# dmMaze/comic-text-detector

Hardware: NVIDIA H100
Metric: pages/sec @1024x1024 synthetic (higher is better)
Workload: dtype fp16

## Files before the change

### comic-text-detector_b200/csrc/conv_tc.cu

```cuda
#include <cstdlib>
#include <cstring>
#include <cuda.h>
#include <cuda_fp16.h>
#include <cuda_runtime.h>

#include "kernels.h"
#include "ptx.cuh"

namespace ctd {

constexpr int kTileW = 16;
constexpr int kThreads = 384;

template <int BN, int TH>
struct TcCfg {
  static constexpr int kABytes = TH * kTileW * 128;
  static constexpr int kBBytes = BN * 128;
  static constexpr int kStages = TH == 8 ? (BN >= 128 ? 5 : (BN >= 64 ? 8 : 10))
                                         : (BN >= 128 ? 3 : (BN >= 64 ? 4 : (BN >= 32 ? 5 : 6)));
  static constexpr int kBoxN = BN < 64 ? BN : 64;
  static constexpr int kBoxBytes = 8 * TH * kBoxN * 2;
  static constexpr int kStgBytes = (BN / kBoxN) * kBoxBytes;
  static constexpr int kBiasFloats = 512;
  static constexpr size_t kSmem = 1024 + size_t(kStages) * (kABytes + kBBytes) + 2 * kStgBytes + 256 + kBiasFloats * 4;
  static_assert(kSmem <= 227 * 1024, "conv_tc_kernel: shared memory");
  static_assert(kBoxBytes % 1024 == 0, "conv_tc_kernel: store boxes must keep the 1024-byte swizzle alignment");
};

template <int ACT>
__device__ __forceinline__ float apply_act(float v) {
  if constexpr (ACT == CTD_ACT_SILU) return __fdividef(v, 1.0f + exp_neg_fast(v));
  else if constexpr (ACT == CTD_ACT_LEAKY) return fmaxf(v, 0.1f * v);
  else if constexpr (ACT == CTD_ACT_RELU) return fmaxf(v, 0.f);
  else if constexpr (ACT == CTD_ACT_SIGMOID) return __fdividef(1.0f, 1.0f + exp_neg_fast(v));
  else return v;
}

template <int ACT>
__device__ __forceinline__ float apply_act_precise(float v) {
  if constexpr (ACT == CTD_ACT_SILU) return v / (1.0f + expf(-v));
  else if constexpr (ACT == CTD_ACT_LEAKY) return fmaxf(v, 0.1f * v);
  else if constexpr (ACT == CTD_ACT_RELU) return fmaxf(v, 0.f);
  else if constexpr (ACT == CTD_ACT_SIGMOID) return 1.0f / (1.0f + expf(-v));
  else return v;
}

template <int BN>
__device__ __forceinline__ void wgmma_bn(float (&d)[BN / 2], uint64_t ad, uint64_t bd, uint32_t acc) {
  if constexpr (BN == 128) wgmma_n128(d, ad, bd, acc);
  else if constexpr (BN == 64) wgmma_n64(d, ad, bd, acc);
  else if constexpr (BN == 32) wgmma_n32(d, ad, bd, acc);
  else wgmma_n16(d, ad, bd, acc);
}

template <int BN, int TH, int ACT, bool RES>
__device__ __forceinline__ void stage_f16(const float (&acc)[BN / 2], const float* __restrict__ bias_s, uint32_t stg,
                                          int m, int warp4, int lane) {
  using Cfg = TcCfg<BN, TH>;
  constexpr uint32_t kRowBytes = Cfg::kBoxN * 2;
  const int q = lane >> 3;
  const uint32_t pixrow = uint32_t(m * 64 + warp4 * 16 + (q & 1) * 8 + (lane & 7));
#pragma unroll
  for (int j = 0; j < BN / 8; j += 2) {
    const int col = (j + (q >> 1)) * 8;
    const uint32_t off = pixrow * kRowBytes + uint32_t(col % Cfg::kBoxN) * 2;
    const uint32_t addr = stg + uint32_t(col / Cfg::kBoxN) * Cfg::kBoxBytes +
                          (off ^ (((off >> 7) & (kRowBytes / 16 - 1)) << 4));
    uint32_t r[4];
    if constexpr (RES) ldmatrix_x4(addr, r);
#pragma unroll
    for (int i = 0; i < 4; ++i) {
      const int c = (j + (i >> 1)) * 8 + (lane & 3) * 2;
      float f0 = apply_act<ACT>(acc[j * 4 + 2 * i] + bias_s[c]);
      float f1 = apply_act<ACT>(acc[j * 4 + 2 * i + 1] + bias_s[c + 1]);
      if constexpr (RES) {
        __half2 h;
        memcpy(&h, &r[i], 4);
        const float2 rv = __half22float2(h);
        f0 = __fadd_rn(f0, rv.x);
        f1 = __fadd_rn(f1, rv.y);
      }
      const __half2 o = __floats2half2_rn(f0, f1);
      memcpy(&r[i], &o, 4);
    }
    stmatrix_x4(addr, r);
  }
}

template <int ACT>
__device__ __forceinline__ void epi_pair_f32(float v0, float v1, const float* __restrict__ bias_s, int col,
                                             float* __restrict__ out, int ncols, bool residual) {
  if (col >= ncols) return;
  float f0 = apply_act_precise<ACT>(v0 + bias_s[col]);
  float f1 = apply_act_precise<ACT>(v1 + bias_s[col + 1]);
  if (col + 1 < ncols) {
    if (residual) {
      const float2 r = *reinterpret_cast<const float2*>(out + col);
      f0 += r.x;
      f1 += r.y;
    }
    *reinterpret_cast<float2*>(out + col) = make_float2(f0, f1);
  } else {
    if (residual) f0 += out[col];
    out[col] = f0;
  }
}

template <int BN, int ACT>
__device__ __forceinline__ void epilogue_f32(const float (&acc)[BN / 2], const float* __restrict__ bias_s,
                                             float* const (&out)[2], const bool (&valid)[2], int ncols, int lane,
                                             bool residual) {
#pragma unroll
  for (int h = 0; h < 2; ++h) {
    if (!valid[h]) continue;
#pragma unroll
    for (int j = 0; j < BN / 8; ++j)
      epi_pair_f32<ACT>(acc[j * 4 + 2 * h], acc[j * 4 + 2 * h + 1], bias_s, j * 8 + (lane & 3) * 2, out[h], ncols,
                        residual);
  }
// ... 167 lines not shown
      int prev = -1;
      for (int k_it = 0; k_it < its_per_tile; ++k_it) {
        mbar_wait(full_bar + 8 * stage, full_par);
        const uint64_t ad = a_desc0 + uint64_t(stage) * (Cfg::kABytes >> 4);
        const uint64_t bd = b_desc0 + uint64_t(stage) * (Cfg::kBBytes >> 4);
        wgmma_fence();
        for (int ks = 0; ks < ksteps; ++ks)
#pragma unroll
          for (int m = 0; m < MT; ++m)
            wgmma_bn<BN>(acc[m], ad + m * a_mstep + 2 * ks, bd + 2 * ks, (k_it > 0 || ks > 0) ? 1u : 0u);
        wgmma_commit();
        wgmma_wait<1>();
        if (prev >= 0 && wg_leader) mbar_arrive(empty_bar + 8 * prev);
        prev = stage;
        if (++stage == Cfg::kStages) { stage = 0; full_par ^= 1u; }
      }
      wgmma_wait<0>();
#pragma unroll
      for (int m = 0; m < MT; ++m) wgmma_fence_regs(acc[m]);
      if (prev >= 0 && wg_leader) mbar_arrive(empty_bar + 8 * prev);
    }

    const float* bias_t = bias_s + nblk * BN;
    if (nhwc16) {
      if (res16) {
        mbar_wait(res_bar, res_par);
        res_par ^= 1u;
      } else {
        if (wg_leader) tma_store_wait_read();
        named_barrier_sync(epi_bar, 128);
      }
#define CTD_EPI(ACT)                                                                                   \
  _Pragma("unroll") for (int m = 0; m < MT; ++m) {                                                     \
    if (res16) stage_f16<BN, TH, ACT, true>(acc[m], bias_t, stg, m, warp & 3, lane);                   \
    else stage_f16<BN, TH, ACT, false>(acc[m], bias_t, stg, m, warp & 3, lane);                        \
  }
      switch (g.act) {
        case CTD_ACT_SILU: CTD_EPI(CTD_ACT_SILU) break;
        case CTD_ACT_LEAKY: CTD_EPI(CTD_ACT_LEAKY) break;
        case CTD_ACT_RELU: CTD_EPI(CTD_ACT_RELU) break;
        case CTD_ACT_SIGMOID: CTD_EPI(CTD_ACT_SIGMOID) break;
        default: CTD_EPI(CTD_ACT_NONE) break;
      }
#undef CTD_EPI
      fence_proxy_async();
      named_barrier_sync(epi_bar, 128);
      if (wg_leader) {
#pragma unroll
        for (int b = 0; b < BN / Cfg::kBoxN; ++b)
          tma_store_4d(&p.d_map[phase], stg + b * Cfg::kBoxBytes, nblk * BN + b * Cfg::kBoxN, x0, sy0, img);
        tma_store_commit();
      }
      if (p.dst_map_cols < g.cout && p.dst_map_cols < (nblk + 1) * BN) {
#pragma unroll
        for (int m = 0; m < MT; ++m)
#pragma unroll
          for (int h = 0; h < 2; ++h) {
            const int row = (wg * MT + m) * 64 + wrow + 8 * h;
            const int gy = y0 + row / kTileW, gx = x0 + row % kTileW;
            if (gy >= g.gh || gx >= g.gw) continue;
            const int oy = gy * g.out_mul + (phase >> 1), ox = gx * g.out_mul + (phase & 1);
            __half* out = p.dst + (size_t(img) * g.dst_h * g.dst_w + size_t(oy) * g.dst_w + ox) * g.dst_cstride +
                          g.dst_coff;
#pragma unroll
            for (int i = 0; i < R; ++i) {
              if (((i >> 1) & 1) != h) continue;
              const int c = (i >> 2) * 8 + (lane & 3) * 2 + (i & 1), col = nblk * BN + c;
              if (col < p.dst_map_cols || col >= g.cout) continue;
// ... 41 lines not shown
            if (c >= ncols) continue;
            const int col = nblk * BN + c;
            const int a = col / no, o = col - a * no;
            const float s = 1.0f / (1.0f + expf(-(acc[m][i] + bias_t[c])));
            float r;
            if (o == 0) r = (s * 2.0f - 0.5f + float(gx[h])) * p.det_stride;
            else if (o == 1) r = (s * 2.0f - 0.5f + float(gy[h])) * p.det_stride;
            else if (o == 2) r = (s * 2.0f) * (s * 2.0f) * p.anchor_wh[2 * a];
            else if (o == 3) r = (s * 2.0f) * (s * 2.0f) * p.anchor_wh[2 * a + 1];
            else r = s;
            rows[(size_t(a) * g.gh * g.gw + size_t(gy[h]) * g.gw + gx[h]) * no + o] = r;
          }
        }
      } else {
        float* out32[2];
#pragma unroll
        for (int h = 0; h < 2; ++h)
          out32[h] = reinterpret_cast<float*>(p.dst) + pix[h] * g.dst_cstride + g.dst_coff + nblk * BN;
        const bool res = g.residual != 0;
        switch (g.act) {
          case CTD_ACT_SILU: epilogue_f32<BN, CTD_ACT_SILU>(acc[m], bias_t, out32, valid, ncols, lane, res); break;
          case CTD_ACT_LEAKY: epilogue_f32<BN, CTD_ACT_LEAKY>(acc[m], bias_t, out32, valid, ncols, lane, res); break;
          case CTD_ACT_RELU: epilogue_f32<BN, CTD_ACT_RELU>(acc[m], bias_t, out32, valid, ncols, lane, res); break;
          case CTD_ACT_SIGMOID: epilogue_f32<BN, CTD_ACT_SIGMOID>(acc[m], bias_t, out32, valid, ncols, lane, res); break;
          default: epilogue_f32<BN, CTD_ACT_NONE>(acc[m], bias_t, out32, valid, ncols, lane, res); break;
        }
      }
    }
  }
  if (nhwc16 && wg_leader) tma_store_wait_all();
}


static const char* encode_map(PFN_encodeTiled enc, CUtensorMap* m, const void* base, int rank, const cuuint64_t* dims,
                              const cuuint64_t* strides_bytes, const cuuint32_t* box, int kb_elems) {
  cuuint32_t estr[5] = {1, 1, 1, 1, 1};
  const CUtensorMapSwizzle sw = kb_elems == 64 ? CU_TENSOR_MAP_SWIZZLE_128B
                                               : (kb_elems == 32 ? CU_TENSOR_MAP_SWIZZLE_64B : CU_TENSOR_MAP_SWIZZLE_32B);
  CUresult r = enc(m, CU_TENSOR_MAP_DATA_TYPE_FLOAT16, rank, const_cast<void*>(base), dims, strides_bytes, box, estr,
                   CU_TENSOR_MAP_INTERLEAVE_NONE, sw, CU_TENSOR_MAP_L2_PROMOTION_L2_256B,
                   CU_TENSOR_MAP_FLOAT_OOB_FILL_NONE);
  return r == CUDA_SUCCESS ? nullptr : "cuTensorMapEncodeTiled failed";
}

static const char* encode_dst_maps(PFN_encodeTiled enc, ConvTcParams& p, const __half* dst, int bn, int th) {
  const ConvGeom& g = p.g;
  const int boxn = bn < 64 ? bn : 64;
  p.dst_map_cols = g.cout & ~7;
  if (p.dst_map_cols == 0) return "conv_tc: fp16 destination needs at least 8 output channels";
  const cuuint64_t px = cuuint64_t(g.dst_cstride) * 2;
  for (int ph = 0; ph < g.n_phase; ++ph) {
    const int ph_y = ph >> 1, ph_x = ph & 1;
    const char* base = reinterpret_cast<const char*>(dst) + size_t(g.dst_coff) * 2 + (size_t(ph_y) * g.dst_w + ph_x) * px;
    cuuint64_t dims[4] = {cuuint64_t(p.dst_map_cols), cuuint64_t(g.gw), cuuint64_t(g.gh), cuuint64_t(g.n_img)};
    cuuint64_t str[3] = {px * g.out_mul, px * g.dst_w * g.out_mul, px * g.dst_w * g.dst_h};
    cuuint32_t box[4] = {cuuint32_t(boxn), kTileW, cuuint32_t(th / 2), 1};
    if (const char* e = encode_map(enc, &p.d_map[ph], base, 4, dims, str, box, boxn)) return e;
  }
  return nullptr;
}

static int g_num_sms = 132;

static int pick_block_n(int cout_pad) {
  if (cout_pad >= 128 && cout_pad % 128 == 0) return 128;
  if (cout_pad % 64 == 0) return 64;
  if (cout_pad % 32 == 0) return 32;
  return 16;
}

template <int TH>
static size_t smem_for(int bn) {
  switch (bn) {
    case 128: return TcCfg<128, TH>::kSmem;
    case 64: return TcCfg<64, TH>::kSmem;
    case 32: return TcCfg<32, TH>::kSmem;
    default: return TcCfg<16, TH>::kSmem;
  }
}

const char* conv_tc_plan(ConvTcPlan& plan, PFN_encodeTiled enc, const ConvGeom& g, const void* const src_ptr[],
                         const int src_coff[], const void* w16, const float* bias, __half* dst, int split) {
  ConvTcParams& p = plan.p;
  memset(&p, 0, sizeof(p));
  p.g = g;
  p.split = split ? 1 : 0;
  p.split_img_off = g.n_img;
  p.split_row_off = g.n_phase * g.cout_pad;
  const int n_planes = split ? 2 : 1;
  int kb = 64;
  for (int s = 0; s < g.n_src; ++s) {
    if (g.src_c[s] % 64 != 0 && kb > 32) kb = 32;
    if (g.src_c[s] % 32 != 0) kb = 16;
    if (g.src_c[s] % 16 != 0) return "conv_tc: source channels must be a multiple of 16";
    if (src_coff[s] % 8 != 0) return "conv_tc: source channel offset must be a multiple of 8";
// ... 104 lines not shown
```

### comic-text-detector_b200/csrc/engine.cu

```cuda
#include <cuda.h>
#include <cuda_fp16.h>
#include <cuda_runtime.h>
#include <stdarg.h>
#include <stdio.h>
#include <string.h>

#include <algorithm>
#include <cstdlib>
#include <map>
#include <string>
#include <tuple>
#include <vector>

#include "engine.h"

using namespace ctd;

namespace {
thread_local std::string g_create_error;
}

int ctd_fail(ctd_handle* h, int code, const char* fmt, ...) {
  char buf[512];
  va_list ap;
// ... 113 lines not shown
    }                                                                                                    \
  } while (0)
  CKC(cudaSetDevice(cfg->device));
  {
    int lo = 0, hi = 0;
    CKC(cudaDeviceGetStreamPriorityRange(&lo, &hi));
    CKC(cudaStreamCreateWithPriority(&h->stream, cudaStreamNonBlocking, lo));
    CKC(cudaStreamCreateWithPriority(&h->side, cudaStreamNonBlocking, hi));
    CKC(cudaStreamCreateWithPriority(&h->side2, cudaStreamNonBlocking, hi));
  }
  CKC(cudaEventCreateWithFlags(&h->ev_fork, cudaEventDisableTiming));
  CKC(cudaEventCreateWithFlags(&h->ev_join, cudaEventDisableTiming));
  CKC(cudaEventCreateWithFlags(&h->ev_fork2, cudaEventDisableTiming));
  CKC(cudaEventCreateWithFlags(&h->ev_xjoin, cudaEventDisableTiming));
  CKC(cudaEventCreateWithFlags(&h->ev_join2, cudaEventDisableTiming));
  CKC(cudaEventCreateWithFlags(&h->ev_tin, cudaEventDisableTiming));
  CKC(cudaEventCreateWithFlags(&h->ev_tout, cudaEventDisableTiming));
  CKC(cudaEventCreate(&h->ev0));
  CKC(cudaEventCreate(&h->ev1));
  CKC(cudaEventCreate(&h->tev0));
  CKC(cudaEventCreate(&h->tev1));
  {
    void* fn = nullptr;
    cudaDriverEntryPointQueryResult qres;
    CKC(cudaGetDriverEntryPoint("cuTensorMapEncodeTiled", &fn, cudaEnableDefault, &qres));
    if (!fn || qres != cudaDriverEntryPointSuccess) {
      ctd_fail(h, CTD_E_CUDA, "cuTensorMapEncodeTiled not available from the driver");
      return bail(CTD_E_CUDA);
    }
    h->enc = reinterpret_cast<PFN_encodeTiled>(fn);
  }
  CKC(conv_tc_init());
  CKC(conv_ends_init());
  h->blob_bytes = blob_bytes;
  CKC(cudaMalloc(&h->d_blob, blob_bytes));
  CKC(cudaMemcpy(h->d_blob, blob, blob_bytes, cudaMemcpyHostToDevice));
  const size_t nb = size_t(cfg->max_batch), mh = cfg->max_h, mw = cfg->max_w;
  h->d_buf.assign(n_bufs, nullptr);
  for (int i = 0; i < n_bufs; ++i) {
    const size_t bytes = nb * (mh / bufs[i].down) * (mw / bufs[i].down + 4) * bufs[i].channels * h->elem;
    CKC(cudaMalloc(&h->d_buf[i], bytes));
    CKC(cudaMemset(h->d_buf[i], 0, bytes));
  }
  if (cfg->precision == CTD_PREC_SPLIT_TC) {
    h->d_buf16.assign(n_bufs, nullptr);
    for (int i = 0; i < n_bufs; ++i) {
      const size_t bytes = 2 * nb * (mh / bufs[i].down) * (mw / bufs[i].down + 4) * bufs[i].channels * 2;
      CKC(cudaMalloc(&h->d_buf16[i], bytes));
      CKC(cudaMemset(h->d_buf16[i], 0, bytes));
    }
    h->wsplit_off.assign(size_t(n_ops), 0);
    std::vector<__half> ws;
    const char* hb = static_cast<const char*>(blob);
    for (int i = 0; i < n_ops; ++i) {
      const ctd_op& op = ops[i];
      if (!is_gemm(op.kind)) continue;
      int cin = 0;
      for (int k = 0; k < op.n_src; ++k) cin += op.src_c[k];
      const int taps = op.kind == CTD_OP_DECONV4 ? 4 : op.ksize * op.ksize;
      const int nph = op.kind == CTD_OP_DECONV4 ? 4 : 1;
      const size_t cnt = size_t(nph) * op.cout_pad * taps * cin;
      if (size_t(op.w32_off) + cnt * 4 > blob_bytes || size_t(op.w16_off) + cnt * 2 > blob_bytes) {
        ctd_fail(h, CTD_E_INVALID, "op %d: weights outside the blob", i);
        return bail(CTD_E_INVALID);
      }
      while (ws.size() % 128) ws.push_back(__float2half(0.f));
// ... 73 lines not shown
  g.cout = op.cout;
  g.cout_pad = op.cout_pad;
  if (op.dst_buf >= 0) {
    g.dst_cstride = h->bufs[op.dst_buf].channels;
    g.dst_coff = op.dst_coff;
  }
  g.act = op.act;
  g.residual = op.residual;
  return CTD_OK;
}

template <typename P>
static void set_detect(const ctd_handle* h, size_t i, int ph, int pw, P& p) {
  p.blks = h->d_blks;
  p.blks_rows_per_img = rows_per_image(ph, pw);
  int row0 = 0;
  for (int l = 0; l < h->ops[i].aux; ++l) row0 += 3 * (ph / (8 << l)) * (pw / (8 << l));
  p.level_row0 = row0;
  p.nc = h->cfg.nc;
  p.det_stride = h->detect_prm[i][0];
  for (int k = 0; k < 6; ++k) p.anchor_wh[k] = h->detect_prm[i][1 + k];
}

static bool runs_on_tensor_cores(int precision, int kind) {
  switch (precision) {
    case CTD_PREC_SPLIT_TC: return is_gemm(kind);
    case CTD_PREC_FP16_TC: return is_gemm(kind) || kind == CTD_OP_STEM || kind == CTD_OP_SEG_TAIL;
    default: return false;
  }
}

static int build_plans(ctd_handle* h, int n, int ph, int pw, ShapePlan& sp) {
  sp.tc.resize(h->ops.size());
  sp.ends.resize(h->ops.size());
  const bool split = h->cfg.precision == CTD_PREC_SPLIT_TC;
  for (size_t i = 0; i < h->ops.size(); ++i) {
    const ctd_op& op = h->ops[i];
    if (!runs_on_tensor_cores(h->cfg.precision, op.kind)) continue;
    const float* bias = reinterpret_cast<const float*>(h->d_blob + op.b_off);
    const char* e = nullptr;
    if (op.kind == CTD_OP_STEM) {
      const bool f16 = sp.input == INPUT_F32;
      e = conv_ends_plan_stem(sp.ends[i], h->enc, f16 ? static_cast<const void*>(h->in_stage.p) : h->d_pages, f16, n,
                              ph, pw, h->d_blob + op.w16_off, bias, static_cast<__half*>(h->d_buf[op.dst_buf]),
                              h->bufs[op.dst_buf].channels, op.dst_coff, op.cout, op.act);
    } else if (op.kind == CTD_OP_SEG_TAIL) {
      if (op.cout_pad != 16) return ctd_fail(h, CTD_E_INVALID, "op %zu: seg tail needs cout_pad 16", i);
      const ctd_bufdesc& sb = h->bufs[op.src_buf[0]];
      e = conv_ends_plan_seg(sp.ends[i], h->enc, static_cast<const __half*>(h->d_buf[op.src_buf[0]]), sb.channels,
                             op.src_coff[0], op.src_c[0], n, ph / sb.down, pw / sb.down, h->d_blob + op.w16_off,
                             h->d_mask, h->d_mask_u8);
    } else {
      ConvGeom g;
      if (int rc = op_geom(h, op, n, ph, pw, g)) return rc;
      const void* src[CTD_MAX_SRC];
      int coff[CTD_MAX_SRC];
      for (int s = 0; s < op.n_src; ++s) {
        src[s] = (split ? h->d_buf16 : h->d_buf)[op.src_buf[s]];
        coff[s] = op.src_coff[s];
      }
      const void* w = split ? h->d_wsplit + h->wsplit_off[i] : h->d_blob + op.w16_off;
      __half* dst = op.kind == CTD_OP_DETECT ? nullptr : static_cast<__half*>(h->d_buf[op.dst_buf]);
      e = conv_tc_plan(sp.tc[i], h->enc, g, src, coff, w, bias, dst, split);
      if (op.kind == CTD_OP_DETECT) set_detect(h, i, ph, pw, sp.tc[i].p);
    }
    if (e) return ctd_fail(h, CTD_E_INVALID, "op %zu: %s", i, e);
  }
  return CTD_OK;
}

template <typename T>
static int run_op_simt(ctd_handle* h, size_t i, int n, int ph, int pw) {
  const ctd_op& op = h->ops[i];
  ConvSimtParams p;
  memset(&p, 0, sizeof(p));
  if (int rc = op_geom(h, op, n, ph, pw, p.g)) return rc;
  for (int k = 0; k < op.n_src; ++k)
    p.src[k] = static_cast<char*>(h->d_buf[op.src_buf[k]]) + size_t(op.src_coff[k]) * sizeof(T);
  p.w = h->d_blob + (sizeof(T) == 4 ? op.w32_off : op.w16_off);
  p.bias = reinterpret_cast<const float*>(h->d_blob + op.b_off);
  if (op.kind == CTD_OP_DETECT) set_detect(h, i, ph, pw, p);
  else p.dst = h->d_buf[op.dst_buf];
  CK(conv_simt_launch<T>(p, h->stream));
  return CTD_OK;
}

template <typename T>
static int run_op_thin(ctd_handle* h, const ctd_op& op, int n, int ph, int pw, int input) {
  cudaStream_t s = h->stream;
  const ctd_bufdesc* sb = op.kind == CTD_OP_STEM ? nullptr : &h->bufs[op.src_buf[0]];
  const int sh = sb ? ph / sb->down : ph, sw = sb ? pw / sb->down : pw;
  const T* src = sb ? static_cast<const T*>(h->d_buf[op.src_buf[0]]) + op.src_coff[0] : nullptr;
  switch (op.kind) {
    case CTD_OP_STEM: {
      const float* w = reinterpret_cast<const float*>(h->d_blob + op.w32_off);
      const float* b = reinterpret_cast<const float*>(h->d_blob + op.b_off);
// ... 18 lines not shown
    case CTD_OP_UPSAMPLE2:
      CK(upsample2_launch<T>(src, n, sh, sw, op.src_c[0], sb->channels,
                             static_cast<T*>(h->d_buf[op.dst_buf]) + op.dst_coff, h->bufs[op.dst_buf].channels, s));
      return CTD_OK;
    case CTD_OP_SEG_TAIL:
      CK(seg_tail_launch<T>(src, n, sh, sw, op.src_c[0], sb->channels,
                            reinterpret_cast<const float*>(h->d_blob + op.p_off), h->d_mask, h->d_mask_u8, s));
      return CTD_OK;
    case CTD_OP_DB_TAIL:
      CK(db_tail_launch<T>(src, n, sh, sw, sb->channels, reinterpret_cast<const float*>(h->d_blob + op.p_off),
                           h->d_lines, h->d_bitmap, h->cfg.db_thresh, s));
      return CTD_OK;
    default: return ctd_fail(h, CTD_E_INVALID, "run_op_thin: bad kind %d", op.kind);
  }
}

static int split_written_slice(ctd_handle* h, const ctd_op& op, int n, int ph, int pw, int* cnt) {
  int buf = op.dst_buf, coff = op.dst_coff, c = op.cout;
  if (op.kind == CTD_OP_SPPF_POOL) { buf = op.src_buf[0]; coff = op.src_coff[0] + op.src_c[0]; c = 3 * op.src_c[0]; }
  else if (op.kind == CTD_OP_AVGPOOL2 || op.kind == CTD_OP_UPSAMPLE2) c = op.src_c[0];
  if (buf < 0 || c <= 0) return CTD_OK;
  const ctd_bufdesc& b = h->bufs[buf];
  const size_t npix = size_t(n) * (ph / b.down) * (pw / b.down);
  __half* hi = static_cast<__half*>(h->d_buf16[buf]) + coff;
  CK(split_planes_launch(static_cast<const float*>(h->d_buf[buf]) + coff, hi, hi + npix * b.channels, npix, c, b.channels,
                         h->stream));
  ++*cnt;
  return CTD_OK;
}

static int run_one_op(ctd_handle* h, size_t i, int n, int ph, int pw, const ShapePlan& sp, int* cnt) {
  const ctd_op& op = h->ops[i];
  const ConvTcPlan& tc = sp.tc[i];
  int rc = CTD_OK;
  if (tc.block_n || sp.ends[i].kind != ctd::CTD_END_NONE) {
    const cudaError_t e = tc.block_n ? conv_tc_launch(tc, h->stream) : conv_ends_launch(sp.ends[i], h->stream);
    if (e != cudaSuccess) rc = ctd_fail(h, CTD_E_CUDA, "tensor-core op %zu: %s", i, cudaGetErrorString(e));
  } else if (is_gemm(op.kind)) {
    rc = h->elem == 4 ? run_op_simt<float>(h, i, n, ph, pw) : run_op_simt<__half>(h, i, n, ph, pw);
  } else {
    rc = h->elem == 4 ? run_op_thin<float>(h, op, n, ph, pw, sp.input) : run_op_thin<__half>(h, op, n, ph, pw, sp.input);
  }
  ++*cnt;
  if (rc || h->d_buf16.empty()) return rc;
  return split_written_slice(h, op, n, ph, pw, cnt);
}

int launch_nms(ctd_handle* h, int n, int ph, int pw, cudaStream_t s, int* cnt) {
  CK(nms_launch(h->d_blks, n, rows_per_image(ph, pw), h->cfg.nc, h->cfg.conf_thresh, h->cfg.nms_thresh, h->nms, h->d_det,
                h->d_det_count, s));
  *cnt += kNmsLaunches;
  return CTD_OK;
}

int launch_db_post(ctd_handle* h, int n, int ph, int pw, cudaStream_t s, int* cnt) {
  CK(ccl_launch(h->d_bitmap, n, ph, pw, h->d_labels, h->d_ccl_scratch, h->d_nlabels, s));
  CK(segrep_launch(h->d_bitmap, h->d_lines, size_t(2) * ph * pw, h->d_ccl_scratch, n, ph, pw, 1000, 1.5f,
                   h->d_segrep_scratch, h->d_line_boxes, h->d_line_scores, h->d_line_count, s));
  *cnt += kCclLaunches + kSegrepLaunches;
  return CTD_OK;
}

static int run_ops(ctd_handle* h, int n, int ph, int pw, const ShapePlan& sp, int* launches, bool record = false) {
  int cnt = 0;
  size_t evi = 0;
  if (h->overlap && !record && !h->cfg.debug_skip_postproc) {
    for (size_t i = 0; i < h->ops.size(); ++i)
      if (h->db_ancestor[i])
        if (int rc = run_one_op(h, i, n, ph, pw, sp, &cnt)) return rc;
// ... 478 lines not shown
```

### comic-text-detector_b200/csrc/engine.h

```cpp
#pragma once
#include <cuda.h>
#include <cuda_runtime.h>
#include <stdint.h>

#include <math.h>

#include <algorithm>
#include <array>
#include <condition_variable>
#include <deque>
#include <map>
#include <mutex>
#include <optional>
#include <string>
#include <thread>
#include <tuple>
#include <vector>

#include "kernels.h"

using ctd::ConvTcPlan;
using ctd::ConvEndsPlan;
using ctd::NmsWorkspace;
using ctd::PFN_encodeTiled;

struct ArenaLayout {
  size_t det, cnt, nl, lb, ls, lc, a_bytes, refined, blocks, blocks_stride, rec_off, lines_off, dist_off, total;
};

struct BlockSection {
  size_t rec_off, lines_off, dist_off, stride;
};
inline BlockSection block_section_layout() {
  auto al = [](size_t v) { return (v + 255) / 256 * 256; };
  BlockSection b;
  b.rec_off = 64;
  b.lines_off = b.rec_off + al(size_t(CTD_MAX_BLOCKS) * sizeof(ctd_block));
  b.dist_off = b.lines_off + al(size_t(CTD_MAX_BLOCKS) * 32);
  b.stride = b.dist_off + al(size_t(CTD_MAX_BLOCK_DIST) * 8);
  return b;
}

struct Letterbox {
  int unpad_h, unpad_w;
  float ratio_x, ratio_y;
};
inline bool letterbox_of(int ih, int iw, int net_h, int net_w, Letterbox& lb) {
  if (ih < 1 || iw < 1 || net_h < 1 || net_w < 1) return false;
  const double r = std::min(double(net_h) / ih, double(net_w) / iw);
  lb.unpad_w = int(nearbyint(iw * r));
  lb.unpad_h = int(nearbyint(ih * r));
  if (lb.unpad_w < 1 || lb.unpad_h < 1 || lb.unpad_w > net_w || lb.unpad_h > net_h) return false;
  lb.ratio_x = float(double(iw) / double(lb.unpad_w));
  lb.ratio_y = float(double(ih) / double(lb.unpad_h));
  return true;
// ... 73 lines not shown

  void start(bool want_crops, bool want_on_device, bool want_masks = true) {
    crops = want_crops;
    on_device = want_on_device;
    masks = want_masks;
    collected = false;
  }
  void release();
};

struct RefineJob {
  std::vector<ctd::RefineWin> wins;
  std::vector<ctd::RefineChunk> chunks;
  size_t total_px = 0;
  size_t total_words = 0;
  void add(int x1, int y1, int x2, int y2, size_t page_off, int iw, int ih);
  size_t table_bytes() const;
};

struct RegionJob {
  std::vector<ctd::RegionDev> regs;
  std::vector<ctd::RegionTile> tiles;
  size_t out_bytes = 0;
  int add(const ctd_region* plan, int n, const ctd::RegionPage& pg, long long out_base);
  size_t table_bytes() const;
  void write_tables(char* dst) const;
};

enum { INPUT_U8 = 0, INPUT_F32 = 1 };

struct ShapePlan {
  int input = INPUT_U8;
  std::vector<ConvTcPlan> tc;
  std::vector<ConvEndsPlan> ends;
  cudaGraphExec_t graph = nullptr;
  int launches = 0;
};
struct ctd_handle {
  ctd_config cfg{};
  std::vector<ctd_op> ops;
  std::vector<ctd_bufdesc> bufs;
  std::vector<std::array<float, 7>> detect_prm;
  std::string err;
  cudaStream_t stream = nullptr;
  cudaEvent_t ev0 = nullptr, ev1 = nullptr, tev0 = nullptr, tev1 = nullptr;
  std::vector<cudaEvent_t> op_events;
  PFN_encodeTiled enc = nullptr;
  char* d_blob = nullptr;
  size_t blob_bytes = 0;
  std::vector<void*> d_buf;
  std::vector<void*> d_buf16;
  char* d_wsplit = nullptr;
  std::vector<size_t> wsplit_off;
  int elem = 2;
  uint8_t* d_pages = nullptr;
  float* d_blks = nullptr;
  float* d_mask = nullptr;
  uint8_t* d_mask_u8 = nullptr;
  float* d_lines = nullptr;
  uint8_t* d_bitmap = nullptr;
  float* d_det = nullptr;
  int* d_det_count = nullptr;
  int32_t* d_labels = nullptr;
  int32_t* d_nlabels = nullptr;
  int32_t* d_ccl_scratch = nullptr;
  void* d_segrep_scratch = nullptr;
// ... 53 lines not shown
```

### comic-text-detector_b200/csrc/kernels.h

```cpp
#pragma once
#include <cuda.h>
#include <cuda_fp16.h>
#include <cuda_runtime.h>
#include <stdint.h>

#include "../../include/ctd_b200.h"

namespace ctd {

constexpr int kMaxTaps = 9;

constexpr float kSplitLoScale = 2048.0f;
constexpr float kSplitLoUnscale = 1.0f / 2048.0f;
constexpr int kMaxPhases = 4;

struct ConvGeom {
  int n_img;
  int gh, gw;
  int dst_h, dst_w;
  int out_mul;
  int n_phase;
  int taps;
  int cin_total;
  int k_total;
// ... 21 lines not shown
  int tiles_x, tiles_y;
  int8_t tap_map[kMaxPhases][kMaxTaps];
  __half* dst;
  int dst_map_cols;
  const float* bias;
  float* blks;
  int blks_rows_per_img;
  int level_row0;
  float det_stride;
  float anchor_wh[6];
  int nc;
  int split;
  int split_img_off;
  int split_row_off;
};
static_assert(sizeof(ConvTcParams) <= 4096, "ConvTcParams: kernel parameters are limited to 4 KB");

struct ConvTcPlan {
  ConvTcParams p;
  int block_n;
  int tile_h;
  dim3 grid;
  size_t smem_bytes;
};

typedef CUresult (*PFN_encodeTiled)(CUtensorMap*, CUtensorMapDataType, cuuint32_t, void*, const cuuint64_t*,
                                    const cuuint64_t*, const cuuint32_t*, const cuuint32_t*, CUtensorMapInterleave,
                                    CUtensorMapSwizzle, CUtensorMapL2promotion, CUtensorMapFloatOOBfill);

const char* conv_tc_plan(ConvTcPlan& plan, PFN_encodeTiled enc, const ConvGeom& g, const void* const src_ptr[],
                         const int src_coff[], const void* w16, const float* bias, __half* dst, int split = 0);
cudaError_t conv_tc_launch(const ConvTcPlan& plan, cudaStream_t s);
cudaError_t conv_tc_init();

enum { CTD_END_NONE = 0, CTD_END_STEM = 1, CTD_END_SEG = 2, CTD_END_STEM_F16 = 3 };
struct alignas(64) ConvEndsParams {
  CUtensorMap a_map;
  CUtensorMap b_map;
  CUtensorMap d_map;
  int n_img, gh, gw;
  int tiles_x, tiles_y;
  const float* bias;
  float* mask_f32;
  uint8_t* mask_u8;
};
struct ConvEndsPlan {
  ConvEndsParams p;
  int kind = CTD_END_NONE;
  dim3 grid;
  size_t smem_bytes;
};
const char* conv_ends_plan_stem(ConvEndsPlan& plan, PFN_encodeTiled enc, const void* pages, bool f16_page, int n,
                                int ph, int pw, const void* w16, const float* bias, __half* dst, int dst_cstride,
                                int dst_coff, int cout, int act);
const char* conv_ends_plan_seg(ConvEndsPlan& plan, PFN_encodeTiled enc, const __half* src, int src_cstride,
                               int src_coff, int src_c, int n, int gh, int gw, const void* w16, float* mask_f32,
                               uint8_t* mask_u8);
cudaError_t conv_ends_launch(const ConvEndsPlan& plan, cudaStream_t s);
cudaError_t conv_ends_init();

struct ConvSimtParams {
  ConvGeom g;
  const void* src[CTD_MAX_SRC];
  const void* w;
  const float* bias;
  void* dst;
// ... 131 lines not shown
```

Before: 1172.

## Add persistent 1x1 conv kernel with resident weights and dual-ring TMA pipeline

Adds a dedicated persistent warp-specialized kernel for 1x1 convolutions (no residual, stride 1, single phase). It loads each block's full weight slice into shared memory once, then streams spatial tiles through two independent producer rings, one per consumer warpgroup, so each warpgroup runs its own tile with TMA stores. The aim is to remove repeated weight reloads and per-tile launch/scheduling overhead of the generic conv kernel for pointwise layers. It adds a second code path and moves shared epilogue helpers into a common header. Layers whose weights exceed 64 KB, or that need too many N blocks, fall back to the generic kernel.

```diff
diff --git a/comic-text-detector_b200/csrc/conv_1x1.cu b/comic-text-detector_b200/csrc/conv_1x1.cu
--- /dev/null
+++ b/comic-text-detector_b200/csrc/conv_1x1.cu
@@ -0,0 +1,263 @@
+#include <cstdlib>
+#include <cstring>
+#include <cuda.h>
+#include <cuda_fp16.h>
+#include <cuda_runtime.h>
+
+#include "conv_epi.cuh"
+#include "kernels.h"
+#include "ptx.cuh"
+
+namespace ctd {
+
+namespace {
+
+constexpr int kThreads = 384;
+constexpr int kTileH = 8;
+constexpr int kABytes = 16 * 1024;
+constexpr int kWeightBytes = 64 * 1024;
+
+template <int BN>
+struct C1Cfg {
+  using Box = StoreBox<BN, kTileH>;
+  static constexpr int kStages = BN == 128 ? 3 : 4;
+  static constexpr size_t kSmem =
+      1024 + kWeightBytes + 2 * size_t(kStages) * kABytes + 2 * Box::kStgBytes + 256 + BN * 4;
+  static_assert(kSmem <= 227 * 1024, "conv1x1_tc_kernel: shared memory");
+  static_assert(8 * (4 * kStages + 1) <= 256, "conv1x1_tc_kernel: barriers");
+};
+
+}
+
+template <int BN>
+__global__ void __launch_bounds__(kThreads, 1) conv1x1_tc_kernel(const __grid_constant__ Conv1x1Params p) {
+  using Cfg = C1Cfg<BN>;
+  using Box = typename Cfg::Box;
+  constexpr int S = Cfg::kStages;
+  extern __shared__ __align__(1024) uint8_t smem_c1[];
+  const uint32_t raw_base = smem_u32(smem_c1);
+  const uint32_t smem_base = (raw_base + 1023u) & ~1023u;
+  uint8_t* const smem_gen = smem_c1 + (smem_base - raw_base);
+  const uint32_t w_base = smem_base;
+  const uint32_t a_base = w_base + kWeightBytes;
+  const uint32_t stg_base = a_base + 2 * S * kABytes;
+  const uint32_t bar_base = stg_base + 2 * Box::kStgBytes;
+  const uint32_t full_bar = bar_base, empty_bar = bar_base + 16 * S, w_bar = bar_base + 32 * S;
+  float* bias_s = reinterpret_cast<float*>(smem_gen + (bar_base - smem_base) + 256);
+
+  const int warp = threadIdx.x >> 5, lane = threadIdx.x & 31;
+  const int kb = p.kb_elems;
+  const uint32_t row_bytes = kb * 2;
+  const uint32_t w_blk_bytes = uint32_t(BN) * row_bytes;
+  int kits = 0;
+  for (int s = 0; s < p.n_src; ++s) kits += p.src_kblocks[s];
+  const int n_tiles = [&] {
+    const int first = blockIdx.x / p.n_nblk, step = gridDim.x / p.n_nblk, total = p.n_img * p.tiles_x * p.tiles_y;
+    return first < total ? (total - first + step - 1) / step : 0;
+  }();
+
+  if (warp == 0 && lane == 0) {
+    for (int s = 0; s < p.n_src; ++s) prefetch_tensormap(&p.a_map[s]);
+    prefetch_tensormap(&p.w_map);
+    prefetch_tensormap(&p.d_map);
+    for (int s = 0; s < 2 * S; ++s) {
+      mbar_init(full_bar + 8 * s, 1);
+      mbar_init(empty_bar + 8 * s, 1);
+    }
+    mbar_init(w_bar, 1);
+    fence_barrier_init();
+  }
+  for (int i = threadIdx.x; i < BN; i += kThreads) bias_s[i] = p.bias ? p.bias[(blockIdx.x % p.n_nblk) * BN + i] : 0.f;
+  __syncthreads();
+
+  auto decode = [&](int j, int& img, int& y0, int& x0) {
+    const int sp = blockIdx.x / p.n_nblk + j * (gridDim.x / p.n_nblk);
+    const int tiles_per_img = p.tiles_x * p.tiles_y;
+    img = sp / tiles_per_img;
+    const int r = sp - img * tiles_per_img;
+    const int ty = r / p.tiles_x;
+    y0 = ty * kTileH;
+    x0 = (r - ty * p.tiles_x) * kTileW;
+  };
+
+  if (warp < 4) {
+    setmaxnreg_dec<40>();
+    if (warp < 2 && elect_one()) {
+      const int ring = warp;
+      if (ring == 0) {
+        mbar_arrive_expect_tx(w_bar, uint32_t(kits) * w_blk_bytes);
+        for (int i = 0; i < kits; ++i) tma_load_2d(w_base + i * w_blk_bytes, &p.w_map, w_bar, i * kb,
+                                              (blockIdx.x % p.n_nblk) * BN);
+      }
+      const uint32_t a_tx = uint32_t(16 * kTileH) * row_bytes;
+      int it = 0;
+      for (int j = ring; j < n_tiles; j += 2) {
+        int img, y0, x0;
+        decode(j, img, y0, x0);
+        for (int s = 0; s < p.n_src; ++s) {
+          for (int cb = 0; cb < p.src_kblocks[s]; ++cb, ++it) {
+            const int stage = ring * S + it % S;
+            const uint32_t par = ((it / S) & 1) ^ 1;
+            mbar_wait_relaxed(empty_bar + 8 * stage, par);
+            mbar_arrive_expect_tx(full_bar + 8 * stage, a_tx);
+            tma_load_4d(a_base + stage * kABytes, &p.a_map[s], full_bar + 8 * stage, cb * kb, x0, y0, img);
+          }
+        }
+      }
+    }
+    return;
+  }
+
+  setmaxnreg_inc<232>();
+  const int wg = (warp >> 2) - 1;
+  const bool wg_leader = (threadIdx.x & 127) == 0;
+  const uint64_t a_desc0 = make_kmajor_desc(a_base + uint32_t(wg * S) * kABytes, row_bytes);
+  const uint64_t w_desc0 = make_kmajor_desc(w_base, row_bytes);
+  const uint64_t a_mstep = (64u * row_bytes) >> 4;
+  const int ksteps = kb / 16;
+  const uint32_t stg = stg_base + uint32_t(wg) * Box::kStgBytes;
+  const uint32_t epi_bar = 1 + wg;
+  constexpr int R = BN / 2;
+  int stage = 0;
+  uint32_t full_par = 0;
+  mbar_wait(w_bar, 0);
+
+  const uint32_t my_full = full_bar + 8u * uint32_t(wg * S), my_empty = empty_bar + 8u * uint32_t(wg * S);
+  for (int j = wg; j < n_tiles; j += 2) {
+    float acc[2][R];
+#pragma unroll
+    for (int m = 0; m < 2; ++m)
+#pragma unroll
+      for (int i = 0; i < R; ++i) acc[m][i] = 0.f;
+
+    int prev = -1;
+    for (int k = 0; k < kits; ++k) {
+      mbar_wait(my_full + 8 * stage, full_par);
+      const uint64_t ad = a_desc0 + uint64_t(stage) * (kABytes >> 4);
+      const uint64_t bd = w_desc0 + uint32_t(k) * (w_blk_bytes >> 4);
+      wgmma_fence();
+      for (int ks = 0; ks < ksteps; ++ks)
+#pragma unroll
+        for (int m = 0; m < 2; ++m)
+          wgmma_bn<BN>(acc[m], ad + m * a_mstep + 2 * ks, bd + 2 * ks, (k > 0 || ks > 0) ? 1u : 0u);
+      wgmma_commit();
+      wgmma_wait<1>();
+      if (prev >= 0 && wg_leader) mbar_arrive(my_empty + 8 * prev);
+      prev = stage;
+      if (++stage == S) { stage = 0; full_par ^= 1u; }
+    }
+    wgmma_wait<0>();
+#pragma unroll
+    for (int m = 0; m < 2; ++m) wgmma_fence_regs(acc[m]);
+    if (prev >= 0 && wg_leader) mbar_arrive(my_empty + 8 * prev);
+
+    if (wg_leader) tma_store_wait_read();
+    named_barrier_sync(epi_bar, 128);
+#define CTD_EPI(ACT) \
+  _Pragma("unroll") for (int m = 0; m < 2; ++m) stage_f16<BN, kTileH, ACT, false>(acc[m], bias_s, stg, m, warp & 3, lane);
+    switch (p.act) {
+      case CTD_ACT_SILU: CTD_EPI(CTD_ACT_SILU) break;
+      case CTD_ACT_LEAKY: CTD_EPI(CTD_ACT_LEAKY) break;
+      case CTD_ACT_RELU: CTD_EPI(CTD_ACT_RELU) break;
+      case CTD_ACT_SIGMOID: CTD_EPI(CTD_ACT_SIGMOID) break;
+      default: CTD_EPI(CTD_ACT_NONE) break;
+    }
+#undef CTD_EPI
+    fence_proxy_async();
+    named_barrier_sync(epi_bar, 128);
+    if (wg_leader) {
+      int img, y0, x0;
+      decode(j, img, y0, x0);
+#pragma unroll
+      for (int b = 0; b < BN / Box::kBoxN; ++b)
+        tma_store_4d(&p.d_map, stg + b * Box::kBoxBytes, (blockIdx.x % p.n_nblk) * BN + b * Box::kBoxN, x0, y0, img);
+      tma_store_commit();
+    }
+  }
+  if (wg_leader) tma_store_wait_all();
+}
+
+
+constexpr int kMaxNBlocks = 8;
+
+int conv1x1_block_n(const ConvGeom& g) {
+  if (g.taps != 1 || g.in_stride != 1 || g.n_phase != 1 || g.residual != 0 || g.cout % 8 != 0) return 0;
+  for (int bn = 128; bn >= 16; bn /= 2)
+    if (g.cout_pad % bn == 0 && size_t(g.k_total) * bn * 2 <= size_t(kWeightBytes))
+      return g.cout_pad / bn <= kMaxNBlocks ? bn : 0;
+  return 0;
+}
+
+const char* conv1x1_plan(Conv1x1Plan& plan, PFN_encodeTiled enc, const ConvGeom& g, const void* const src_ptr[],
+                         const int src_coff[], const void* w16, const float* bias, __half* dst) {
+  Conv1x1Params& p = plan.p;
+  memset(&p, 0, sizeof(p));
+  const int bn = conv1x1_block_n(g);
+  if (bn == 0) return "conv1x1: op outside the kernel's class";
+  int kb = 64;
+  for (int s = 0; s < g.n_src; ++s) {
+    if (g.src_c[s] % 64 != 0 && kb > 32) kb = 32;
+    if (g.src_c[s] % 32 != 0) kb = 16;
+    if (g.src_c[s] % 16 != 0) return "conv1x1: source channels must be a multiple of 16";
+    if (src_coff[s] % 8 != 0) return "conv1x1: source channel offset must be a multiple of 8";
+  }
+  if ((g.dst_coff % 8) != 0 || (g.dst_cstride % 8) != 0) return "conv1x1: destination slice must be 16-byte aligned";
+  p.n_src = g.n_src;
+  p.kb_elems = kb;
+  for (int s = 0; s < g.n_src; ++s) p.src_kblocks[s] = g.src_c[s] / kb;
+  p.n_img = g.n_img;
+  p.tiles_x = (g.gw + kTileW - 1) / kTileW;
+  p.tiles_y = (g.gh + kTileH - 1) / kTileH;
+  p.n_nblk = g.cout_pad / bn;
+  p.act = g.act;
+  p.bias = bias;
+  for (int s = 0; s < g.n_src; ++s) {
+    const size_t cs = size_t(g.src_cstride[s]);
+    const char* base = static_cast<const char*>(src_ptr[s]) + size_t(src_coff[s]) * 2;
+    cuuint64_t dims[4] = {cuuint64_t(g.src_c[s]), cuuint64_t(g.src_w), cuuint64_t(g.src_h), cuuint64_t(g.n_img)};
+    cuuint64_t str[3] = {cs * 2, cs * 2 * g.src_w, cs * 2 * g.src_w * g.src_h};
+    cuuint32_t box[4] = {cuuint32_t(kb), kTileW, kTileH, 1};
+    if (const char* e = encode_map(enc, &p.a_map[s], base, 4, dims, str, box, kb)) return e;
+  }
+  {
+    cuuint64_t dims[2] = {cuuint64_t(g.k_total), cuuint64_t(g.cout_pad)};
+    cuuint64_t str[1] = {cuuint64_t(g.k_total) * 2};
+    cuuint32_t box[2] = {cuuint32_t(kb), cuuint32_t(bn)};
+    if (const char* e = encode_map(enc, &p.w_map, w16, 2, dims, str, box, kb)) return e;
+  }
+  if (const char* e = encode_dst_map(enc, &p.d_map, g, 0, dst, bn, kTileH)) return e;
+  const int spatial = g.n_img * p.tiles_x * p.tiles_y;
+  int per_nblk = conv_sm_count() / p.n_nblk;
+  if (per_nblk > spatial) per_nblk = spatial;
+  plan.grid = dim3(unsigned(per_nblk * p.n_nblk), 1, 1);
+  plan.block_n = bn;
+  switch (bn) {
+    case 128: plan.smem_bytes = C1Cfg<128>::kSmem; break;
+    case 64: plan.smem_bytes = C1Cfg<64>::kSmem; break;
+    case 32: plan.smem_bytes = C1Cfg<32>::kSmem; break;
+    default: plan.smem_bytes = C1Cfg<16>::kSmem; break;
+  }
+  return nullptr;
+}
+
+cudaError_t conv1x1_init() {
+  cudaError_t e;
+#define CTD_SET(BN)                                                                                               \
+  e = cudaFuncSetAttribute(conv1x1_tc_kernel<BN>, cudaFuncAttributeMaxDynamicSharedMemorySize, int(C1Cfg<BN>::kSmem)); \
+  if (e != cudaSuccess) return e;
+  CTD_SET(128) CTD_SET(64) CTD_SET(32) CTD_SET(16)
+#undef CTD_SET
+  return cudaSuccess;
+}
+
+cudaError_t conv1x1_launch(const Conv1x1Plan& plan, cudaStream_t s) {
+  switch (plan.block_n) {
+    case 128: conv1x1_tc_kernel<128><<<plan.grid, kThreads, plan.smem_bytes, s>>>(plan.p); break;
+    case 64: conv1x1_tc_kernel<64><<<plan.grid, kThreads, plan.smem_bytes, s>>>(plan.p); break;
+    case 32: conv1x1_tc_kernel<32><<<plan.grid, kThreads, plan.smem_bytes, s>>>(plan.p); break;
+    default: conv1x1_tc_kernel<16><<<plan.grid, kThreads, plan.smem_bytes, s>>>(plan.p); break;
+  }
+  return cudaGetLastError();
+}
+
+}
diff --git a/comic-text-detector_b200/csrc/conv_epi.cuh b/comic-text-detector_b200/csrc/conv_epi.cuh
--- /dev/null
+++ b/comic-text-detector_b200/csrc/conv_epi.cuh
@@ -0,0 +1,71 @@
+#pragma once
+#include <cstring>
+#include <cuda_fp16.h>
+
+#include "kernels.h"
+#include "ptx.cuh"
+
+namespace ctd {
+
+constexpr int kTileW = 16;
+
+template <int BN, int ROWS>
+struct StoreBox {
+  static constexpr int kBoxN = BN < 64 ? BN : 64;
+  static constexpr int kBoxBytes = ROWS * kTileW * kBoxN * 2;
+  static constexpr int kStgBytes = (BN / kBoxN) * kBoxBytes;
+  static_assert(kBoxBytes % 1024 == 0, "store boxes must keep the 1024-byte swizzle alignment");
+};
+
+template <int ACT>
+__device__ __forceinline__ float apply_act(float v) {
+  if constexpr (ACT == CTD_ACT_SILU) return __fdividef(v, 1.0f + exp_neg_fast(v));
+  else if constexpr (ACT == CTD_ACT_LEAKY) return fmaxf(v, 0.1f * v);
+  else if constexpr (ACT == CTD_ACT_RELU) return fmaxf(v, 0.f);
+  else if constexpr (ACT == CTD_ACT_SIGMOID) return __fdividef(1.0f, 1.0f + exp_neg_fast(v));
+  else return v;
+}
+
+template <int BN>
+__device__ __forceinline__ void wgmma_bn(float (&d)[BN / 2], uint64_t ad, uint64_t bd, uint32_t acc) {
+  if constexpr (BN == 128) wgmma_n128(d, ad, bd, acc);
+  else if constexpr (BN == 64) wgmma_n64(d, ad, bd, acc);
+  else if constexpr (BN == 32) wgmma_n32(d, ad, bd, acc);
+  else wgmma_n16(d, ad, bd, acc);
+}
+
+template <int BN, int ROWS, int ACT, bool RES>
+__device__ __forceinline__ void stage_f16(const float (&acc)[BN / 2], const float* __restrict__ bias_s, uint32_t stg,
+                                          int m, int warp4, int lane) {
+  using Box = StoreBox<BN, ROWS>;
+  constexpr uint32_t kRowBytes = Box::kBoxN * 2;
+  const int q = lane >> 3;
+  const uint32_t pixrow = uint32_t(m * 64 + warp4 * 16 + (q & 1) * 8 + (lane & 7));
+#pragma unroll
+  for (int j = 0; j < BN / 8; j += 2) {
+    const int col = (j + (q >> 1)) * 8;
+    const uint32_t off = pixrow * kRowBytes + uint32_t(col % Box::kBoxN) * 2;
+    const uint32_t addr = stg + uint32_t(col / Box::kBoxN) * Box::kBoxBytes +
+                          (off ^ (((off >> 7) & (kRowBytes / 16 - 1)) << 4));
+    uint32_t r[4];
+    if constexpr (RES) ldmatrix_x4(addr, r);
+#pragma unroll
+    for (int i = 0; i < 4; ++i) {
+      const int c = (j + (i >> 1)) * 8 + (lane & 3) * 2;
+      float f0 = apply_act<ACT>(acc[j * 4 + 2 * i] + bias_s[c]);
+      float f1 = apply_act<ACT>(acc[j * 4 + 2 * i + 1] + bias_s[c + 1]);
+      if constexpr (RES) {
+        __half2 h;
+        memcpy(&h, &r[i], 4);
+        const float2 rv = __half22float2(h);
+        f0 = __fadd_rn(f0, rv.x);
+        f1 = __fadd_rn(f1, rv.y);
+      }
+      const __half2 o = __floats2half2_rn(f0, f1);
+      memcpy(&r[i], &o, 4);
+    }
+    stmatrix_x4(addr, r);
+  }
+}
+
+}
diff --git a/comic-text-detector_b200/csrc/conv_tc.cu b/comic-text-detector_b200/csrc/conv_tc.cu
--- a/comic-text-detector_b200/csrc/conv_tc.cu
+++ b/comic-text-detector_b200/csrc/conv_tc.cu
@@ -4,12 +4,12 @@
 #include <cuda_fp16.h>
 #include <cuda_runtime.h>
 
+#include "conv_epi.cuh"
 #include "kernels.h"
 #include "ptx.cuh"
 
 namespace ctd {
 
-constexpr int kTileW = 16;
 constexpr int kThreads = 384;
 
 template <int BN, int TH>
@@ -18,23 +18,13 @@
   static constexpr int kBBytes = BN * 128;
   static constexpr int kStages = TH == 8 ? (BN >= 128 ? 5 : (BN >= 64 ? 8 : 10))
                                          : (BN >= 128 ? 3 : (BN >= 64 ? 4 : (BN >= 32 ? 5 : 6)));
-  static constexpr int kBoxN = BN < 64 ? BN : 64;
-  static constexpr int kBoxBytes = 8 * TH * kBoxN * 2;
-  static constexpr int kStgBytes = (BN / kBoxN) * kBoxBytes;
+  static constexpr int kBoxN = StoreBox<BN, TH / 2>::kBoxN;
+  static constexpr int kBoxBytes = StoreBox<BN, TH / 2>::kBoxBytes;
+  static constexpr int kStgBytes = StoreBox<BN, TH / 2>::kStgBytes;
   static constexpr int kBiasFloats = 512;
   static constexpr size_t kSmem = 1024 + size_t(kStages) * (kABytes + kBBytes) + 2 * kStgBytes + 256 + kBiasFloats * 4;
   static_assert(kSmem <= 227 * 1024, "conv_tc_kernel: shared memory");
-  static_assert(kBoxBytes % 1024 == 0, "conv_tc_kernel: store boxes must keep the 1024-byte swizzle alignment");
 };
-
-template <int ACT>
-__device__ __forceinline__ float apply_act(float v) {
-  if constexpr (ACT == CTD_ACT_SILU) return __fdividef(v, 1.0f + exp_neg_fast(v));
-  else if constexpr (ACT == CTD_ACT_LEAKY) return fmaxf(v, 0.1f * v);
-  else if constexpr (ACT == CTD_ACT_RELU) return fmaxf(v, 0.f);
-  else if constexpr (ACT == CTD_ACT_SIGMOID) return __fdividef(1.0f, 1.0f + exp_neg_fast(v));
-  else return v;
-}
 
 template <int ACT>
 __device__ __forceinline__ float apply_act_precise(float v) {
@@ -43,48 +33,6 @@
   else if constexpr (ACT == CTD_ACT_RELU) return fmaxf(v, 0.f);
   else if constexpr (ACT == CTD_ACT_SIGMOID) return 1.0f / (1.0f + expf(-v));
   else return v;
-}
-
-template <int BN>
-__device__ __forceinline__ void wgmma_bn(float (&d)[BN / 2], uint64_t ad, uint64_t bd, uint32_t acc) {
-  if constexpr (BN == 128) wgmma_n128(d, ad, bd, acc);
-  else if constexpr (BN == 64) wgmma_n64(d, ad, bd, acc);
-  else if constexpr (BN == 32) wgmma_n32(d, ad, bd, acc);
-  else wgmma_n16(d, ad, bd, acc);
-}
-
-template <int BN, int TH, int ACT, bool RES>
-__device__ __forceinline__ void stage_f16(const float (&acc)[BN / 2], const float* __restrict__ bias_s, uint32_t stg,
-                                          int m, int warp4, int lane) {
-  using Cfg = TcCfg<BN, TH>;
-  constexpr uint32_t kRowBytes = Cfg::kBoxN * 2;
-  const int q = lane >> 3;
-  const uint32_t pixrow = uint32_t(m * 64 + warp4 * 16 + (q & 1) * 8 + (lane & 7));
-#pragma unroll
-  for (int j = 0; j < BN / 8; j += 2) {
-    const int col = (j + (q >> 1)) * 8;
-    const uint32_t off = pixrow * kRowBytes + uint32_t(col % Cfg::kBoxN) * 2;
-    const uint32_t addr = stg + uint32_t(col / Cfg::kBoxN) * Cfg::kBoxBytes +
-                          (off ^ (((off >> 7) & (kRowBytes / 16 - 1)) << 4));
-    uint32_t r[4];
-    if constexpr (RES) ldmatrix_x4(addr, r);
-#pragma unroll
-    for (int i = 0; i < 4; ++i) {
-      const int c = (j + (i >> 1)) * 8 + (lane & 3) * 2;
-      float f0 = apply_act<ACT>(acc[j * 4 + 2 * i] + bias_s[c]);
-      float f1 = apply_act<ACT>(acc[j * 4 + 2 * i + 1] + bias_s[c + 1]);
-      if constexpr (RES) {
-        __half2 h;
-        memcpy(&h, &r[i], 4);
-        const float2 rv = __half22float2(h);
-        f0 = __fadd_rn(f0, rv.x);
-        f1 = __fadd_rn(f1, rv.y);
-      }
-      const __half2 o = __floats2half2_rn(f0, f1);
-      memcpy(&r[i], &o, 4);
-    }
-    stmatrix_x4(addr, r);
-  }
 }
 
 template <int ACT>
@@ -318,8 +266,8 @@
       }
 #define CTD_EPI(ACT)                                                                                   \
   _Pragma("unroll") for (int m = 0; m < MT; ++m) {                                                     \
-    if (res16) stage_f16<BN, TH, ACT, true>(acc[m], bias_t, stg, m, warp & 3, lane);                   \
-    else stage_f16<BN, TH, ACT, false>(acc[m], bias_t, stg, m, warp & 3, lane);                        \
+    if (res16) stage_f16<BN, TH / 2, ACT, true>(acc[m], bias_t, stg, m, warp & 3, lane);                   \
+    else stage_f16<BN, TH / 2, ACT, false>(acc[m], bias_t, stg, m, warp & 3, lane);                        \
   }
       switch (g.act) {
         case CTD_ACT_SILU: CTD_EPI(CTD_ACT_SILU) break;
@@ -427,8 +375,8 @@
 }
 
 
-static const char* encode_map(PFN_encodeTiled enc, CUtensorMap* m, const void* base, int rank, const cuuint64_t* dims,
-                              const cuuint64_t* strides_bytes, const cuuint32_t* box, int kb_elems) {
+const char* encode_map(PFN_encodeTiled enc, CUtensorMap* m, const void* base, int rank, const cuuint64_t* dims,
+                       const cuuint64_t* strides_bytes, const cuuint32_t* box, int kb_elems) {
   cuuint32_t estr[5] = {1, 1, 1, 1, 1};
   const CUtensorMapSwizzle sw = kb_elems == 64 ? CU_TENSOR_MAP_SWIZZLE_128B
                                                : (kb_elems == 32 ? CU_TENSOR_MAP_SWIZZLE_64B : CU_TENSOR_MAP_SWIZZLE_32B);
@@ -438,24 +386,29 @@
   return r == CUDA_SUCCESS ? nullptr : "cuTensorMapEncodeTiled failed";
 }
 
+const char* encode_dst_map(PFN_encodeTiled enc, CUtensorMap* m, const ConvGeom& g, int ph, const __half* dst, int bn,
+                           int box_rows) {
+  const int boxn = bn < 64 ? bn : 64;
+  const cuuint64_t px = cuuint64_t(g.dst_cstride) * 2;
+  const int ph_y = ph >> 1, ph_x = ph & 1;
+  const char* base = reinterpret_cast<const char*>(dst) + size_t(g.dst_coff) * 2 + (size_t(ph_y) * g.dst_w + ph_x) * px;
+  cuuint64_t dims[4] = {cuuint64_t(g.cout & ~7), cuuint64_t(g.gw), cuuint64_t(g.gh), cuuint64_t(g.n_img)};
+  cuuint64_t str[3] = {px * g.out_mul, px * g.dst_w * g.out_mul, px * g.dst_w * g.dst_h};
+  cuuint32_t box[4] = {cuuint32_t(boxn), kTileW, cuuint32_t(box_rows), 1};
+  return encode_map(enc, m, base, 4, dims, str, box, boxn);
+}
+
 static const char* encode_dst_maps(PFN_encodeTiled enc, ConvTcParams& p, const __half* dst, int bn, int th) {
-  const ConvGeom& g = p.g;
-  const int boxn = bn < 64 ? bn : 64;
-  p.dst_map_cols = g.cout & ~7;
+  p.dst_map_cols = p.g.cout & ~7;
   if (p.dst_map_cols == 0) return "conv_tc: fp16 destination needs at least 8 output channels";
-  const cuuint64_t px = cuuint64_t(g.dst_cstride) * 2;
-  for (int ph = 0; ph < g.n_phase; ++ph) {
-    const int ph_y = ph >> 1, ph_x = ph & 1;
-    const char* base = reinterpret_cast<const char*>(dst) + size_t(g.dst_coff) * 2 + (size_t(ph_y) * g.dst_w + ph_x) * px;
-    cuuint64_t dims[4] = {cuuint64_t(p.dst_map_cols), cuuint64_t(g.gw), cuuint64_t(g.gh), cuuint64_t(g.n_img)};
-    cuuint64_t str[3] = {px * g.out_mul, px * g.dst_w * g.out_mul, px * g.dst_w * g.dst_h};
-    cuuint32_t box[4] = {cuuint32_t(boxn), kTileW, cuuint32_t(th / 2), 1};
-    if (const char* e = encode_map(enc, &p.d_map[ph], base, 4, dims, str, box, boxn)) return e;
-  }
+  for (int ph = 0; ph < p.g.n_phase; ++ph)
+    if (const char* e = encode_dst_map(enc, &p.d_map[ph], p.g, ph, dst, bn, th / 2)) return e;
   return nullptr;
 }
 
 static int g_num_sms = 132;
+
+int conv_sm_count() { return g_num_sms; }
 
 static int pick_block_n(int cout_pad) {
   if (cout_pad >= 128 && cout_pad % 128 == 0) return 128;
diff --git a/comic-text-detector_b200/csrc/engine.cu b/comic-text-detector_b200/csrc/engine.cu
--- a/comic-text-detector_b200/csrc/engine.cu
+++ b/comic-text-detector_b200/csrc/engine.cu
@@ -169,6 +169,7 @@
   }
   CKC(conv_tc_init());
   CKC(conv_ends_init());
+  CKC(conv1x1_init());
   h->blob_bytes = blob_bytes;
   CKC(cudaMalloc(&h->d_blob, blob_bytes));
   CKC(cudaMemcpy(h->d_blob, blob, blob_bytes, cudaMemcpyHostToDevice));
@@ -308,6 +309,7 @@
 
 static int build_plans(ctd_handle* h, int n, int ph, int pw, ShapePlan& sp) {
   sp.tc.resize(h->ops.size());
+  sp.c1.resize(h->ops.size());
   sp.ends.resize(h->ops.size());
   const bool split = h->cfg.precision == CTD_PREC_SPLIT_TC;
   for (size_t i = 0; i < h->ops.size(); ++i) {
@@ -337,7 +339,10 @@
       }
       const void* w = split ? h->d_wsplit + h->wsplit_off[i] : h->d_blob + op.w16_off;
       __half* dst = op.kind == CTD_OP_DETECT ? nullptr : static_cast<__half*>(h->d_buf[op.dst_buf]);
-      e = conv_tc_plan(sp.tc[i], h->enc, g, src, coff, w, bias, dst, split);
+      if (!split && op.kind == CTD_OP_CONV && conv1x1_block_n(g) != 0)
+        e = conv1x1_plan(sp.c1[i], h->enc, g, src, coff, w, bias, dst);
+      else
+        e = conv_tc_plan(sp.tc[i], h->enc, g, src, coff, w, bias, dst, split);
       if (op.kind == CTD_OP_DETECT) set_detect(h, i, ph, pw, sp.tc[i].p);
     }
     if (e) return ctd_fail(h, CTD_E_INVALID, "op %zu: %s", i, e);
@@ -422,9 +427,12 @@
 static int run_one_op(ctd_handle* h, size_t i, int n, int ph, int pw, const ShapePlan& sp, int* cnt) {
   const ctd_op& op = h->ops[i];
   const ConvTcPlan& tc = sp.tc[i];
+  const Conv1x1Plan& c1 = sp.c1[i];
   int rc = CTD_OK;
-  if (tc.block_n || sp.ends[i].kind != ctd::CTD_END_NONE) {
-    const cudaError_t e = tc.block_n ? conv_tc_launch(tc, h->stream) : conv_ends_launch(sp.ends[i], h->stream);
+  if (tc.block_n || c1.block_n || sp.ends[i].kind != ctd::CTD_END_NONE) {
+    const cudaError_t e = tc.block_n   ? conv_tc_launch(tc, h->stream)
+                          : c1.block_n ? conv1x1_launch(c1, h->stream)
+                                       : conv_ends_launch(sp.ends[i], h->stream);
     if (e != cudaSuccess) rc = ctd_fail(h, CTD_E_CUDA, "tensor-core op %zu: %s", i, cudaGetErrorString(e));
   } else if (is_gemm(op.kind)) {
     rc = h->elem == 4 ? run_op_simt<float>(h, i, n, ph, pw) : run_op_simt<__half>(h, i, n, ph, pw);
diff --git a/comic-text-detector_b200/csrc/engine.h b/comic-text-detector_b200/csrc/engine.h
--- a/comic-text-detector_b200/csrc/engine.h
+++ b/comic-text-detector_b200/csrc/engine.h
@@ -21,6 +21,7 @@
 
 using ctd::ConvTcPlan;
 using ctd::ConvEndsPlan;
+using ctd::Conv1x1Plan;
 using ctd::NmsWorkspace;
 using ctd::PFN_encodeTiled;
 
@@ -160,6 +161,7 @@
 struct ShapePlan {
   int input = INPUT_U8;
   std::vector<ConvTcPlan> tc;
+  std::vector<Conv1x1Plan> c1;
   std::vector<ConvEndsPlan> ends;
   cudaGraphExec_t graph = nullptr;
   int launches = 0;
diff --git a/comic-text-detector_b200/csrc/kernels.h b/comic-text-detector_b200/csrc/kernels.h
--- a/comic-text-detector_b200/csrc/kernels.h
+++ b/comic-text-detector_b200/csrc/kernels.h
@@ -77,6 +77,35 @@
                          const int src_coff[], const void* w16, const float* bias, __half* dst, int split = 0);
 cudaError_t conv_tc_launch(const ConvTcPlan& plan, cudaStream_t s);
 cudaError_t conv_tc_init();
+int conv_sm_count();
+const char* encode_map(PFN_encodeTiled enc, CUtensorMap* m, const void* base, int rank, const cuuint64_t* dims,
+                       const cuuint64_t* strides_bytes, const cuuint32_t* box, int kb_elems);
+const char* encode_dst_map(PFN_encodeTiled enc, CUtensorMap* m, const ConvGeom& g, int ph, const __half* dst, int bn,
+                           int box_rows);
+
+struct alignas(64) Conv1x1Params {
+  CUtensorMap a_map[CTD_MAX_SRC];
+  CUtensorMap w_map;
+  CUtensorMap d_map;
+  int n_src;
+  int kb_elems;
+  int src_kblocks[CTD_MAX_SRC];
+  int n_img, tiles_x, tiles_y;
+  int n_nblk;
+  int act;
+  const float* bias;
+};
+struct Conv1x1Plan {
+  Conv1x1Params p;
+  int block_n = 0;
+  dim3 grid;
+  size_t smem_bytes;
+};
+int conv1x1_block_n(const ConvGeom& g);
+const char* conv1x1_plan(Conv1x1Plan& plan, PFN_encodeTiled enc, const ConvGeom& g, const void* const src_ptr[],
+                         const int src_coff[], const void* w16, const float* bias, __half* dst);
+cudaError_t conv1x1_launch(const Conv1x1Plan& plan, cudaStream_t s);
+cudaError_t conv1x1_init();
 
 enum { CTD_END_NONE = 0, CTD_END_STEM = 1, CTD_END_SEG = 2, CTD_END_STEM_F16 = 3 };
 struct alignas(64) ConvEndsParams {
```

Measured after the change: 1161 (median of 6 runs). About the same (-0.9%).
